# ChristophAl/tsne-flink

Hardware: AMD Instinct MI355X
Metric: t-SNE iterations/sec + end-to-end sec at N=1M×128 on 1/2/4/8 MI355X; kNN pts/s (higher is better)
Workload: dtype f64

## Files before the change

tsne-flink_amd/csrc/bhtree.hip:

```cpp
#include <hipcub/hipcub.hpp>

#include "bhtree_impl.hpp"

namespace tsne {
namespace {

constexpr int STACK = 320;
constexpr int QREC_V4 = sizeof(QRec) / 16;
constexpr int MOM_TASKS = 128;
__host__ __device__ constexpr double fact(int k) { return k <= 1 ? 1.0 : k * fact(k - 1); }
__host__ __device__ constexpr double binom(int k, int i) { return fact(k) / (fact(i) * fact(k - i)); }

__device__ __forceinline__ double recip_bh(double x) {
    const double r = __builtin_amdgcn_rcp(x);
    return __fma_rn(r, __fma_rn(-x, r, 1.0), r);
}

__device__ __forceinline__ void leaf_force(double qx, double qy, double px, double py, double &fx,
                                           double &fy, double &zs) {
    if (px == qx && py == qy) return;
    const double dx = qx - px, dy = qy - py;
    const double D = __fma_rn(dx, dx, dy * dy);
    const double r = recip_bh(1.0 + D);
    const double sc = r * r;
// ... 854 lines not shown
    }
    if (k == 0 && c == 0 && valid) {
        F[s] = make_double2(fx, fy);
        Z[s] = zs;
    }
    if (k == 0 && c == 0) nv.mtask_n[h * 64 + part * NQ + q] = valid ? ntask : 0;
    const int wwant = wave_sum(nwant);
    if (lane == 0) {
        nv.ncost[h * NPARTS + part] = npops + (ntilepts >> 6);
        if (wwant && __hip_atomic_load(&mom_flag[1], __ATOMIC_RELAXED, __HIP_MEMORY_SCOPE_AGENT) < mom_flag[2])
            atomicAdd(&mom_flag[1], wwant);
    }
    if (COST && bcost && __ballot(valid)) {
        const unsigned long long cc = ((unsigned long long)(clock64() - t_start) >> 6) + 1;
        if (cost_lab) {
            if (valid && k == 0 && c == 0) atomicAdd(&bcost[cost_lab[s] >> 8], (cc + NQ - 1) / NQ);
        } else {
            const int64_t sf = wave_min(valid ? s : ((int64_t)1 << 62));
            if (lane == 0) atomicAdd(&bcost[sf >> 8], cc);
        }
    }
    if (STATS && visits) {
        const unsigned long long tv = wave_sum(nvis);
        if (lane == 0) {
            atomicAdd(visits, tv);
            atomicAdd(visits + 3, (unsigned long long)npops);
            atomicAdd(visits + 4, (unsigned long long)ntilepts);
            atomicMax(visits + 8, (unsigned long long)npops);
            atomicAdd(visits + 30, 1ull);
            const unsigned long long w_end = wall_clock64();
            atomicMax(visits + 15, w_end - w_start);
            atomicMax(visits + 16, ~0ull - w_start);
            atomicMax(visits + 17, w_end);
            atomicAdd(visits + 18, w_end - w_start);
            atomicAdd(visits + 37, (unsigned long long)(clock64() - t_start));
            atomicMax(visits + 31, w_end - w_start);
            wave_log_put(nv.wlog, w_start, w_end, 1);
        }
    }
}

template <int MODE>
#ifdef NARROW_WPE
#define NARROW_ATTR __attribute__((amdgpu_waves_per_eu(NARROW_WPE)))
#else
#define NARROW_ATTR
#endif
__global__ __launch_bounds__(256) NARROW_ATTR void bh_traverse_narrow(
    const double2 *__restrict__ pos, const int32_t *__restrict__ dupc, const BHNode *__restrict__ nodes,
    const QRec *__restrict__ qrec, int32_t *__restrict__ ttask_n, const int32_t *__restrict__ meta,
    int32_t *__restrict__ mom_flag, double mom_tol, double theta, int64_t g0, int64_t g1,
    const int32_t *__restrict__ qlist, int32_t virt, double2 *__restrict__ F, double *__restrict__ Z,
// ... 1395 lines not shown
    val[b] = (int32_t)b;
}

int64_t narrow_fill(const tsne_ctx *ctx, int64_t waves) {
    const int64_t cap = 32 * (int64_t)ctx->cu_count;
    if (waves >= cap) return 0;
    return waves < cap / 2 ? waves : (cap - waves) / (NPARTS - 1);
}

}

static void block_order(tsne_ctx *ctx, BHTree &t, const int32_t *cost, int64_t nwaves, int64_t nblocks,
                        int32_t *order) {
    hipStream_t st = ctx->stream;
    hipLaunchKernelGGL(block_cost_keys, dim3(ceil_div(nblocks, 256)), dim3(256), 0, st, cost, nwaves, nblocks, t.okey,
                       t.oval);
    size_t tb = t.osort_tmp_bytes;
    TSNE_HIP(hipcub::DeviceRadixSort::SortPairsDescending(t.osort_tmp, tb, t.okey, t.okey2, t.oval, order,
                                                          (int)nblocks, 0, 32, st));
}

void bh_alloc(tsne_ctx *ctx, BHTree &t, int64_t n, const std::string &pre) {
    Workspace &ws = ctx->ws;
    bh_alloc_tree(ctx, t, n, pre);
    const int64_t qwaves = ceil_div(n, 64) + 4;
    t.tile_waves = qwaves + qwaves / 2 + 64;
    t.mtask = ws.get<int32_t>(pre + "mtask", (size_t)std::max<int64_t>(n, t.tile_waves * 64) * MOM_TASKS);
    t.mtask_n = ws.get<int32_t>(pre + "mtask_n", std::max<int64_t>(n, t.tile_waves * 64));
    t.ttask = ws.get<TileTask>(pre + "ttask", (size_t)t.tile_waves * TILE_CAP);
    t.ttask_n = ws.get<int32_t>(pre + "ttask_n", t.tile_waves);
    bh_alloc_build_tmp(ctx, t, n, pre);
    const int64_t nb = ceil_div(t.tile_waves, 4);
    t.wcost = ws.get<int32_t>(pre + "wcost", t.tile_waves);
    t.tcost = ws.get<int32_t>(pre + "tcost", t.tile_waves);
    t.okey = ws.get<int32_t>(pre + "okey", nb);
    t.okey2 = ws.get<int32_t>(pre + "okey2", nb);
    t.oval = ws.get<int32_t>(pre + "oval", nb);
    t.border = ws.get<int32_t>(pre + "border", nb);
    t.torder = ws.get<int32_t>(pre + "torder", nb);
    size_t ob = 0;
    TSNE_HIP(hipcub::DeviceRadixSort::SortPairsDescending(nullptr, ob, t.okey, t.okey2, t.oval, t.border, (int)nb, 0,
                                                          32, ctx->stream));
    t.osort_tmp_bytes = ob;
    t.osort_tmp = ws.get<uint8_t>(pre + "osort_tmp", ob);
    t.sel_waves = 0;
    t.ran_narrow = false;
// ... 86 lines not shown
    if (!t.sp_ctl) return 0;
    int32_t c[SP_NCTL];
    TSNE_HIP(hipMemcpyAsync(c, t.sp_ctl, sizeof(c), hipMemcpyDeviceToHost, ctx->stream));
    TSNE_HIP(hipStreamSynchronize(ctx->stream));
    return flags ? (int64_t)c[SP_OVF] : (int64_t)c[SP_TASKS];
}

int64_t bh_narrow_groups(tsne_ctx *ctx, BHTree &t) {
    if (!t.ran_narrow || !t.hran) return 0;
    int32_t h = 0;
    TSNE_HIP(hipMemcpyAsync(&h, t.hran, sizeof(int32_t), hipMemcpyDeviceToHost, ctx->stream));
    TSNE_HIP(hipStreamSynchronize(ctx->stream));
    return h;
}

BHTree &bh_single_tree(tsne_ctx *ctx, int64_t n) {
    if (!ctx->single_tree) ctx->single_tree = new BHTree();
    BHTree &t = *ctx->single_tree;
    if (t.n != n) bh_alloc(ctx, t, n, "bh1.");
    if (!ctx->opts.reuse_costs) { t.sel_waves = 0; t.sp_waves = 0; t.front_waves = 0; }
    return t;
}

void bh_repulsion(tsne_ctx *ctx, BHTree &t, double theta, int64_t s0, int64_t s1,
                  double2 *dF, double *dz, unsigned long long *visits, const int32_t *qlist,
                  unsigned long long *bcost, bool cost_by_label, int32_t *plim) {
    if (s1 <= s0) return;
    hipStream_t st = ctx->stream;
    const double mom_tol = ctx->opts.mom_tol;
    if (t.root_tile) {
        if (visits)
            hipLaunchKernelGGL(root_tile_eval<true>, dim3(ceil_div(s1 - s0, 256)), dim3(256), 0, st, t.root_pos,
                               t.nodes, t.rcoef, t.meta, s0, s1, qlist, dF, dz, visits, mom_tol);
        else
            hipLaunchKernelGGL(root_tile_eval<false>, dim3(ceil_div(s1 - s0, 256)), dim3(256), 0, st, t.root_pos,
                               t.nodes, t.rcoef, t.meta, s0, s1, qlist, dF, dz, visits, mom_tol);
        TSNE_LAUNCH_CHECK();
        return;
    }
    const int mode = visits ? 2 : (bcost ? 1 : 0);
    const bool burst = ctx->opts.trav_burst != 0;
    auto kern = plim ? (mode == 2 ? bh_traverse<2, true, false> : mode == 1 ? bh_traverse<1, true, false>
                                                                         : bh_traverse<0, true, false>)
                : burst ? (mode == 2 ? bh_traverse<2, false, false, true> : mode == 1 ? bh_traverse<1, false, false, true>
                                                                                   : bh_traverse<0, false, false, true>)
                        : (mode == 2 ? bh_traverse<2, false, false> : mode == 1 ? bh_traverse<1, false, false>
// ... 35 lines not shown
    const int cblocks = std::max(1, ctx->cu_count * o.tile_stream);
    if (stream) {
        bh_stream_alloc(ctx, t);
        stv.ctl = t.st_ctl;
        stv.gen = ++t.st_gen;
        if (t.st_gen >= (1 << 29)) t.st_gen = 1;
        stv.gen = t.st_gen;
        stv.maxcost = o.tile_stream_max;
        stv.wait = o.tile_stream_wait;
        stv.total = (int32_t)(nblocks * TRAV_WPB);
        stv.cap = (int32_t)t.tile_waves;
        if (!o.tile_stream_gate) {
            TSNE_HIP(hipEventRecord(ctx->st_ev[0], st));
            TSNE_HIP(hipStreamWaitEvent(ctx->st_stream, ctx->st_ev[0], 0));
        }
    }
    t.ran_stream = stream;
    bool mom_late = false;
    if (t.mom_deferred) {
        t.mom_deferred = false;
        if (stream) bh_moments(t, st);
        else mom_late = true;
    }
    if (mom_late && !narrow) {
        TSNE_HIP(hipEventRecord(ctx->aux_ev[0], st));
        TSNE_HIP(hipStreamWaitEvent(ctx->aux_stream, ctx->aux_ev[0], 0));
    }
    stv.prio = o.trav_prio;
    if (o.trav_front > 0.0 && narrow && t.front_waves == waves) stv.border = t.trav_order;
    if (t.order_ready && narrow && !plim && !qlist && s0 == 0 && waves == ceil_div(t.n, 64)) {
        TSNE_HIP(hipStreamWaitEvent(st, t.ord_ev, 0));
        stv.border = t.trav_order;
    }
    stv.wlog = wlog;
    const int32_t *clab = cost_by_label ? t.idx_sorted : nullptr;
    if (narrow) {
        TSNE_HIP(hipEventRecord(ctx->aux_ev[0], st));
        TSNE_HIP(hipStreamWaitEvent(ctx->aux_stream, ctx->aux_ev[0], 0));
        auto nk = mode == 2 ? bh_traverse_narrow<2> : mode == 1 ? bh_traverse_narrow<1> : bh_traverse_narrow<0>;
        hipLaunchKernelGGL(nk, dim3(nv.nbn), dim3(256), 0, ctx->aux_stream, t.pos, t.dupc, t.nodes, t.qrec, t.ttask_n,
                           t.meta, t.mom_flag, mom_tol, theta, s0, s1, qlist, (int32_t)t.n, dF, dz, visits, bcost,
                           t.tcost, clab, nv);
        TSNE_HIP(hipEventRecord(ctx->aux_ev[1], ctx->aux_stream));
    }
    hipLaunchKernelGGL(kern, dim3(nblocks), dim3(64 * TRAV_WPB), 0, st, t.pos, t.dupc, t.nodes, t.qrec, t.ttask, t.ttask_n,
                       t.meta, t.mom_flag, mom_tol, theta, s0, s1, qlist, (int32_t)t.n, dF, dz, visits, bcost, t.wcost,
                       t.tcost, clab, nv, plim, sv, stv);
    if (mom_late) {
        bh_moments(t, ctx->aux_stream);
        if (!t.mom_ev) TSNE_HIP(hipEventCreateWithFlags(&t.mom_ev, hipEventDisableTiming));
        TSNE_HIP(hipEventRecord(t.mom_ev, ctx->aux_stream));
    }
    if (stream) {
        if (o.tile_stream_gate)
            TSNE_HIP(hipStreamWaitValue32(ctx->st_stream, t.st_ctl + ST_STARTED, (uint32_t)nblocks,
                                          hipStreamWaitValueGte, 0xffffffffu));
        ChunkView scv;
        scv.Fp = t.st_Dp;
        scv.Zp = t.st_Dz;
        tile_apply_launch<2>(o.tile_pass, false, visits != nullptr, dim3(cblocks), ctx->st_stream, t.pos, t.nodes, t.ttask,
                             t.ttask_n, s0, s1, qlist, t.mom_flag, mom_tol, t.st_mtask, t.st_mtask_n, dF, dz, visits,
                             (const int32_t *)nullptr, scv, t.mom, SpillView(), stv, t.tcost);
        TSNE_HIP(hipEventRecord(ctx->st_ev[2], st));
        TSNE_HIP(hipStreamWaitEvent(ctx->st_stream, ctx->st_ev[2], 0));
        hipLaunchKernelGGL(stream_finish, dim3(ceil_div((int64_t)stv.total * 64, 256)), dim3(256), 0, ctx->st_stream,
                           t.pos, t.nodes, t.mom, t.st_ctl, t.st_mtask, t.st_mtask_n, t.st_Dp, t.st_Dz, s0, s1,
                           dF, dz, stv.cap, stv.gen);
        TSNE_HIP(hipMemsetAsync(t.st_ctl, 0, sizeof(int32_t) * ST_RESET, ctx->st_stream));
        TSNE_HIP(hipEventRecord(ctx->st_ev[1], ctx->st_stream));
    }
    const int levels = std::min(o.spill_drains, SP_LMAX);
    for (int d = 1; spill && d <= levels; ++d) {
        SpillView dv = sv;
        dv.lin = d;
        dv.lout = d < levels ? d + 1 : 0;
// ... 30 lines not shown
                         t.ttask_n, s0, s1, qlist, t.mom_flag, mom_tol, t.mtask, t.mtask_n, dF, dz, visits, torder, cv,
                         t.mom, SpillView(), stv, t.tcost);
    hipLaunchKernelGGL(moment_apply, dim3(ceil_div(tslots * 64, 256)), dim3(256), 0, st, t.pos, t.nodes, t.mom,
                       t.mtask, t.mtask_n, s0, s1, qlist, dF, dz, cv);
    const bool keep_pcost = o.trav_front_cur > 0.0 && !plim && !qlist && s0 == 0 && s1 == t.n;
    if (keep_pcost) {
        t.pcost = ctx->ws.get<int32_t>(t.pre + "pcost", (size_t)t.n);
        t.pred = ctx->ws.get<int32_t>(t.pre + "pred", (size_t)ceil_div(t.n, 64) + 1);
        t.trav_order = ctx->ws.get<int32_t>(t.pre + "trav_order", ceil_div(t.tile_waves, TRAV_WPB) + 1);
    }
    hipLaunchKernelGGL(chunk_combine, dim3(ceil_div(s1 - s0, 256)), dim3(256), 0, st, t.ch_Fp, t.ch_Zp, t.ch_C,
                       t.ch_slot0, s0, s1, qlist, dF, dz, keep_pcost ? t.pcost : nullptr, t.idx_sorted, t.wcost,
                       narrow ? t.nflag : nullptr);
    t.pcost_valid = keep_pcost;
    if (spill) {
        tile_apply_launch<1>(o.tile_pass, false, visits != nullptr, dim3(std::max(1, ctx->cu_count * 4)), st, t.pos, t.nodes,
                             t.ttask, t.ttask_n, s0, s1, qlist, t.mom_flag, mom_tol, t.mtask, t.mtask_n, dF, dz, visits,
                             (const int32_t *)nullptr, ChunkView(), t.mom, sv, StreamView(), t.tcost);
        hipLaunchKernelGGL(spill_combine, dim3(ceil_div(s1 - s0, 256)), dim3(256), 0, st, t.sp_gflag, t.sp_gen,
                           t.sp_acc, s0, s1, qlist, dF, dz, t.sp_ctl);
    }
    if (narrow) {
        TSNE_HIP(hipStreamWaitEvent(st, ctx->aux_ev[1], 0));
        hipLaunchKernelGGL(narrow_moment_apply, dim3(ceil_div(t.nar_hmax * 64, 256)), dim3(256), 0, st, t.pos,
                           t.nodes, t.mom, t.hlist, t.hcount, t.nmtask, t.nmtask_n, s0, s1, qlist, dF, dz);
        TSNE_HIP(hipMemcpyAsync(t.hran, t.hcount, sizeof(int32_t), hipMemcpyDeviceToDevice, st));
    }
    if (nfac > 0.0 && !plim) {
        if (!narrow) TSNE_HIP(hipMemsetAsync(t.nflag, 0, sizeof(int32_t) * waves, st));
        const bool front = o.trav_front > 0.0;
        if (front) t.trav_order = ctx->ws.get<int32_t>(t.pre + "trav_order", ceil_div(t.tile_waves, TRAV_WPB) + 1);
        hipLaunchKernelGGL(narrow_select, dim3(1), dim3(1024), 0, st, t.wcost, waves, t.nflag, t.ncost, t.hlist,
                           t.hcount, t.nar_hmax, nfac, std::min<int64_t>(t.nar_hmax, narrow_fill(ctx, waves)),
                           front ? t.trav_order : nullptr, o.trav_front);
        t.sel_waves = waves;
        t.front_waves = front ? waves : 0;
    } else {
        t.sel_waves = 0;
        t.front_waves = 0;
    }
    if (o.spill > 0.0 && o.spill_force == 0 && !plim) {
        bh_spill_alloc(ctx, t);
        hipLaunchKernelGGL(spill_budget, dim3(1), dim3(1024), 0, st, t.wcost, waves, o.spill, o.spill_task,
                           (int32_t)o.spill_min, t.sp_ctl);
        t.sp_waves = waves;
    } else {
        t.sp_waves = 0;
    }
    if (stream) TSNE_HIP(hipStreamWaitEvent(st, ctx->st_ev[1], 0));
    TSNE_LAUNCH_CHECK();
}

bool repulsion_stat(tsne_ctx *ctx, const std::string &name, int64_t *value_out) {
    const int at = name == "bh.pops" ? 3 : name == "bh.tile_points" ? 4 : name == "bh.child_slots" ? 6
                 : name == "bh.visits" ? 0 : name == "bh.wave_ticks_max" ? 15 : name == "bh.wave_ticks_sum" ? 18
                 : name == "bh.span_ticks" ? 17 : name == "bh.dense_pairs" ? 2 : name == "bh.moment_evals" ? 1
                 : name == "bh.tile_ticks_max" ? 19 : name == "bh.tile_ticks_sum" ? 22 : name == "bh.tile_span_ticks" ? 21
                 : name == "bh.slow_wave_ticks" ? 33 : name == "bh.slow_wave_pops" ? 33 : name == "bh.slow_wave_ties" ? 34
                 : name == "bh.slow_wave_tile_points" ? 35 : name == "bh.slow_wave_slots" ? 36
                 : name == "bh.wave_mhz" ? 37 : -1;
    int atk = at;
    if (at < 0 && name.size() == 14 && name.compare(0, 13, "bh.tile_steps") == 0) atk = 24 + 2 * (name[13] - '0');
    if (at < 0 && name.size() == 14 && name.compare(0, 13, "bh.tile_pairs") == 0) atk = 25 + 2 * (name[13] - '0');
    if (at < 0 && name.size() == 17 && name.compare(0, 14, "bh.tile_gsteps") == 0 && name[15] == '_' &&
        (name[14] == '0' || name[14] == '1') && (name[16] == '2' || name[16] == '4' || name[16] == '8'))
        atk = (name[14] == '1' ? 38 : 41) + (name[16] == '2' ? 0 : name[16] == '4' ? 1 : 2);
    if (name == "bh.tile_rounds_max") atk = 44;
    if (name == "bh.tile_chunked_waves") atk = 45;
    if (atk < 0 || atk >= VIS_N) return false;
    TSNE_REQUIRE(ctx->opts.rep_stats && ctx->ws.has("rep.visits"), "counter '" + name + "' needs option rep_stats");
    unsigned long long v[VIS_N];
    TSNE_HIP(hipMemcpyAsync(v, ctx->ws.get<unsigned long long>("rep.visits", VIS_N), sizeof(v), hipMemcpyDeviceToHost,
                            ctx->stream));
    TSNE_HIP(hipStreamSynchronize(ctx->stream));
    *value_out = atk == 17 ? (int64_t)(v[17] - (~0ull - v[16])) : atk == 21 ? (int64_t)(v[21] - (~0ull - v[20]))
                                                                              : (int64_t)v[atk];
    if (atk == 37) *value_out = v[18] ? (int64_t)(100.0 * (double)v[37] / (double)v[18]) : 0;
    if (atk >= 33 && atk <= 36)
        *value_out = name == "bh.slow_wave_ticks" ? (int64_t)(v[atk] >> 24) : (int64_t)(v[atk] & ((1ull << 24) - 1));
    return true;
}

}
```

tsne-flink_amd/csrc/bhtree.hpp:

```cpp
#pragma once
#include "common.hpp"
#include "csort.hpp"

namespace tsne {

constexpr int TILE_CAP = 8192;
struct TileTask {
    int32_t ref, first, last, pad;
    uint64_t mask;
};

struct __attribute__((aligned(16))) BHNode {
    double cx, cy;
    double h;
    double hmin;
    double bx0, bx1, by0, by1;
    int32_t cnt;
    int32_t left;
    int32_t right;
    int32_t delta;
    int32_t first, last;
    double rball;
};

// ... 100 lines not shown
    int4 *sp_task = nullptr;
    uint4 *sp_ent = nullptr;
    int32_t *sp_gflag = nullptr;
    unsigned long long *sp_acc = nullptr;
    TileTask *sp_pg_tiles = nullptr;
    int32_t *sp_pg_grp = nullptr, *sp_pg_n = nullptr;
    int32_t sp_cap = 0, sp_pg_cap = 0;
    int32_t sp_gen = 0;
    int64_t sp_waves = 0;
    bool ran_spill = false;
    int32_t *st_ctl = nullptr;
    double2 *st_Dp = nullptr;
    double *st_Dz = nullptr;
    int32_t *st_mtask = nullptr, *st_mtask_n = nullptr;
    int32_t st_gen = 0;
    size_t st_words = 0;
    int32_t *trav_order = nullptr;
    int64_t front_waves = 0;
    int32_t *pcost = nullptr, *pred = nullptr;
    bool pcost_valid = false, order_ready = false;
    hipEvent_t ord_ev = nullptr;
    bool mom_deferred = false;
    hipEvent_t mom_ev = nullptr;
    bool ran_stream = false;
    std::string pre;
};

void bh_alloc(tsne_ctx *ctx, BHTree &t, int64_t n, const std::string &pre = "bh.");
BHTree &bh_single_tree(tsne_ctx *ctx, int64_t n);
void bh_build(tsne_ctx *ctx, BHTree &t, const double *dY, double theta, const int32_t *rowmap = nullptr,
              bool root_tile_ok = false, double near_tol = -1.0);
double bh_near_tol(const tsne_ctx *ctx, bool late);
void bh_repulsion(tsne_ctx *ctx, BHTree &t, double theta, int64_t s0, int64_t s1,
                  double2 *dF, double *dz, unsigned long long *visits, const int32_t *qlist = nullptr,
                  unsigned long long *bcost = nullptr, bool cost_by_label = false, int32_t *plim = nullptr);
void part_align(tsne_ctx *ctx, BHTree &t, const int64_t *cuts, int world, int rank, int32_t *plim);
void part_recut(tsne_ctx *ctx, const unsigned long long *cost, int world, int64_t n, int64_t *cuts);
void part_cost(tsne_ctx *ctx, BHTree &t, int64_t waves, unsigned long long *out);
int64_t bh_spill_counter(tsne_ctx *ctx, BHTree &t, bool flags);
int64_t bh_stream_counter(tsne_ctx *ctx, BHTree &t);
int64_t bh_narrow_groups(tsne_ctx *ctx, BHTree &t);
void bh_balance(tsne_ctx *ctx, const unsigned long long *bcost, int64_t n, int world, int64_t *bounds);

}
```

tsne-flink_amd/csrc/bhtree_build.hip:

```cpp
#include <hipcub/hipcub.hpp>

#include "bhtree_impl.hpp"

namespace tsne {
namespace {

constexpr uint64_t OUT_KEY = MORTON2_OUT_KEY;
constexpr int MOM_CHUNK = 2048;

__global__ void bbox_partial(const double *__restrict__ Y, int64_t n, double *__restrict__ part) {
    __shared__ double sm[4][4];
    double mnx = __builtin_inf(), mxx = -__builtin_inf(), mny = __builtin_inf(), mxy = -__builtin_inf();
    for (int64_t i = (int64_t)blockIdx.x * blockDim.x + threadIdx.x; i < n;
         i += (int64_t)gridDim.x * blockDim.x) {
        double x = Y[2 * i], y = Y[2 * i + 1];
        mnx = fmin(mnx, x); mxx = fmax(mxx, x);
        mny = fmin(mny, y); mxy = fmax(mxy, y);
    }
    mnx = wave_min(mnx); mxx = wave_max(mxx); mny = wave_min(mny); mxy = wave_max(mxy);
    const int w = threadIdx.x >> 6;
    if (lane_id() == 0) { sm[w][0] = mnx; sm[w][1] = mxx; sm[w][2] = mny; sm[w][3] = mxy; }
    __syncthreads();
    if (threadIdx.x == 0) {
        for (int k = 1; k < 4; ++k) {
// ... 1019 lines not shown
    t.status_h = ctx->pinned;
    t.rcoef = ws.get<double>(pre + "rcoef", POLY_K);
    t.dup_mask = ((uint64_t)1 << (64 - __builtin_clzll((uint64_t)std::max<int64_t>(2, 4 * n) - 1))) - 1;
    t.dup_tab = ws.get<int32_t>(pre + "dup_tab", t.dup_mask + 1);
    t.dup_open = ws.get<uint8_t>(pre + "dup_open", n);
    size_t tb = 0;
    morton_sort(nullptr, tb, t.keys, t.keys_sorted, t.idx, t.idx_sorted, n, ctx->stream);
    t.sort_tmp_bytes = tb;
    t.sort_tmp = ws.get<uint8_t>(pre + "sort_tmp", tb);
    csort_alloc(ctx, t.cs, n, pre);
    t.cs_primed = false;
}

double bh_near_tol(const tsne_ctx *ctx, bool late) { return late ? ctx->opts.near_tol_late : ctx->opts.near_tol_early; }

double bh_near_dmax(double theta, double tol) {
    if (!(theta > 0.0)) return __builtin_inf();
    if (!(tol > 0.0)) return -1.0;
    double d = std::sqrt(tol / (48.0 * theta * theta));
    while (48.0 * theta * theta * d * d * (1.0 + 8.0 * d) > tol) d *= 0.99;
    return d;
}

void bh_moments(BHTree &t, hipStream_t ms) {
    const int64_t n = t.n;
    hipLaunchKernelGGL(moment_count, dim3(ceil_div(n + 1, 1024)), dim3(1024), 0, ms, t.nodes, n, t.meta, t.mom_flag,
                       t.mom_cnt, t.mom_list, t.meta, t.mom_off, t.mom_item);
    const int mgrid = (int)std::min<int64_t>(2048, std::max<int64_t>(1, ceil_div(n, 256)));
    hipLaunchKernelGGL(moment_items<true>, dim3(mgrid), dim3(256), 0, ms, t.pos, t.nodes, t.mom_off, n, t.mom_item,
                       t.mom_part, t.mom_cnt, t.mom);
    hipLaunchKernelGGL(moment_reduce, dim3(mgrid), dim3(256), 0, ms, t.meta, t.mom_list, t.mom_cnt, t.mom_off,
                       t.mom_part, t.mom);
}

void bh_build(tsne_ctx *ctx, BHTree &t, const double *dY, double theta, const int32_t *rowmap, bool root_tile_ok,
              double near_tol) {
    if (near_tol < 0.0) near_tol = bh_near_tol(ctx, false);
    t.near_dmax = bh_near_dmax(theta, near_tol);
    hipStream_t st = ctx->stream;
    const int64_t n = t.n;
    t.rowmap = rowmap;
    t.root_tile = false;
    t.mom_deferred = false;
    const bool fuse_opt = ctx->opts.build_fuse != 0;
    if (!fuse_opt) TSNE_HIP(hipMemsetAsync(t.dflag, 0, sizeof(int32_t), st));
    hipLaunchKernelGGL(bbox_partial, dim3(t.bbox_blocks), dim3(256), 0, st, dY, n, t.bbox_part);
    hipLaunchKernelGGL(bbox_final, dim3(1), dim3(256), 0, st, t.bbox_part, t.bbox_blocks, t.W, t.meta, t.bb,
                       t.mom_flag, t.mom_off + n, fuse_opt ? t.dflag : nullptr);
    if (root_tile_ok && t.rt_skip > 0) {
        --t.rt_skip;
        root_tile_ok = false;
    }
    if (root_tile_ok) {
        hipLaunchKernelGGL(root_tile_check, dim3(1), dim3(1), 0, st, t.dflag, t.bb, t.W, n, theta, t.near_dmax,
                           t.status);
        TSNE_HIP(hipMemcpyAsync(t.status_h, t.status, 2 * sizeof(int32_t), hipMemcpyDeviceToHost, st));
        TSNE_HIP(hipStreamSynchronize(st));
        if (!t.status_h[0]) {
            root_tile_ok = false;
            if (t.status_h[1] >= 3) t.rt_skip = std::min(64, 4 * (t.status_h[1] - 2));
        }
    }
    if (root_tile_ok) {
// ... 92 lines not shown
```

tsne-flink_amd/csrc/bhtree_impl.hpp:

```cpp
#pragma once

#include "bhtree.hpp"

namespace tsne {
namespace {

constexpr int MOM_ORDER = 4;
constexpr int MOM_DEG = 2 * MOM_ORDER + 1;
constexpr int MOM_K = (MOM_DEG + 1) * (MOM_DEG + 2) / 2;
constexpr int MOM_MIN_POINTS = 64;
__host__ __device__ constexpr int midx(int a, int b) { return a * (MOM_DEG + 1) - a * (a - 1) / 2 + b; }

__host__ __device__ constexpr int poly_len(int d) { return (d + 1) * (d + 2) / 2; }
__host__ __device__ constexpr int poly_off_z(int i) { return i == 0 ? 0 : poly_off_z(i - 1) + poly_len(2 * i - 2); }
constexpr int POLY_X = poly_off_z(MOM_ORDER + 1);
__host__ __device__ constexpr int poly_off_x(int i) { return i == 0 ? POLY_X : poly_off_x(i - 1) + poly_len(2 * i - 1); }
constexpr int POLY_Y = poly_off_x(MOM_ORDER + 1);
__host__ __device__ constexpr int poly_off_y(int i) { return POLY_Y + poly_off_x(i) - POLY_X; }
constexpr int POLY_K = POLY_Y + (POLY_Y - POLY_X);
static_assert(POLY_K == 345, "MOM_ORDER 4: 95 + 125 + 125 coefficients");

#ifndef TRAV_WPB
#define TRAV_WPB 4
#endif

constexpr int32_t REF_FORCED = 1 << 30;
constexpr int PART_LEVEL = 10;

__device__ __forceinline__ void box_centre(double bx0, double bx1, double by0, double by1, double &cx, double &cy,
                                           double &R) {
    cx = 0.5 * (bx0 + bx1);
    cy = 0.5 * (by0 + by1);
    const double ex = 0.5 * (bx1 - bx0), ey = 0.5 * (by1 - by0);
    R = sqrt(ex * ex + ey * ey) * (1.0 + 1e-12);
}
__device__ __forceinline__ void box_centre(const BHNode &nd, double &cx, double &cy, double &R) {
    box_centre(nd.bx0, nd.bx1, nd.by0, nd.by1, cx, cy, R);
}

}

void bh_moments(BHTree &t, hipStream_t ms);

void bh_alloc_tree(tsne_ctx *ctx, BHTree &t, int64_t n, const std::string &pre);
void bh_alloc_build_tmp(tsne_ctx *ctx, BHTree &t, int64_t n, const std::string &pre);

}
```

tsne-flink_amd/csrc/capi.cpp:

```cpp
#include <cmath>
#include <cstdio>
#include <cstring>
#include <exception>
#include <new>
#include <algorithm>
#include <thread>

#include "bhtree.hpp"
#include "common.hpp"
#include "pca.hpp"
#include "ranks.hpp"
#include "transform.hpp"

namespace tsne {

static thread_local std::string g_last_error;

[[noreturn]] void fail(int status, const std::string &msg) { throw Error(status, msg); }

template <class Fn> static int guard(Fn &&fn) {
    try {
        fn();
        return TSNE_OK;
    } catch (const Error &e) {
// ... 100 lines not shown
    {"spill", &Options::spill, nullptr, 0.0, 1e6},
    {"spill_task", &Options::spill_task, nullptr, 0.0, 1e6},
    {"spill_min", nullptr, &Options::spill_min, 1, 1 << 30},
    {"spill_force", nullptr, &Options::spill_force, 0, 1 << 30},
    {"spill_drains", nullptr, &Options::spill_drains, 1, 8},
    {"tile_stream", nullptr, &Options::tile_stream, 0, 8},
    {"tile_stream_max", nullptr, &Options::tile_stream_max, -1, 1 << 30},
    {"tile_stream_frac", &Options::tile_stream_frac, nullptr, 0.0, 64.0},
    {"tile_stream_gate", nullptr, &Options::tile_stream_gate, 0, 1},
    {"trav_prio", nullptr, &Options::trav_prio, 0, 3},
    {"trav_burst", nullptr, &Options::trav_burst, 0, 1},
    {"trav_front", &Options::trav_front, nullptr, 0.0, 1e6},
    {"trav_front_cur", &Options::trav_front_cur, nullptr, 0.0, 1e6},
    {"wave_log", nullptr, &Options::wave_log, 0, 1},
    {"attract_serial_t0", nullptr, &Options::attract_serial_t0, 0, 1 << 30},
    {"attract_serial_t1", nullptr, &Options::attract_serial_t1, -1, 1 << 30},
    {"tile_stream_wait", nullptr, &Options::tile_stream_wait, 1, 1 << 20},
    {"comm_world1", nullptr, &Options::comm_world1, 0, 1},
    {"rep_stats", nullptr, &Options::rep_stats, 0, 1},
    {"loop_serial", nullptr, &Options::loop_serial, 0, 1},
    {"bu_acqrel", nullptr, &Options::bu_acqrel, 0, 1},
    {"bh_split", nullptr, &Options::bh_split, 0, 1},
    {"build_fuse", nullptr, &Options::build_fuse, 0, 1},
    {"tile_pass", nullptr, &Options::tile_pass, 0, 8},
    {"tile_prefetch", nullptr, &Options::tile_prefetch, 0, 1},
    {"transform_resort", nullptr, &Options::transform_resort, 0, 1 << 30},
    {"transform_split", nullptr, &Options::transform_split, 0, 1},
    {"transform_stats", nullptr, &Options::transform_stats, 0, 1},
};
static const OptionField &option_field(const char *key) {
    for (const OptionField &f : k_options)
        if (std::strcmp(f.key, key) == 0) return f;
    fail(TSNE_ERR_ARG, std::string("unknown option '") + key + "'");
}
static void set_option(Options &o, const char *key, double v) {
    const OptionField &f = option_field(key);
    TSNE_REQUIRE(v >= f.lo && v <= f.hi, std::string("option '") + key + "' out of range");
    if (f.d) o.*f.d = v;
    else {
        TSNE_REQUIRE(v == std::floor(v), std::string("option '") + key + "' takes an integer");
        TSNE_REQUIRE(f.i != &Options::tile_pass || v <= 2 || v == 4 || v == 8, "option 'tile_pass' takes 0, 1, 2, 4 or 8");
        o.*f.i = (int)v;
    }
}
static double get_option(const Options &o, const char *key) {
    const OptionField &f = option_field(key);
// ... 109 lines not shown
        TSNE_REQUIRE(d_bcost != nullptr && d_bounds != nullptr && n >= 0 && world >= 1, "bad balance arguments");
        bh_balance(ctx, reinterpret_cast<const unsigned long long *>(d_bcost), n, world, d_bounds);
    });
}

int tsne_ctx_create(int32_t device, tsne_ctx **out) {
    return guard([&] {
        TSNE_REQUIRE(out != nullptr, "out is NULL");
        *out = nullptr;
        int count = 0;
        if (hipGetDeviceCount(&count) != hipSuccess || count <= 0)
            fail(TSNE_ERR_NO_DEVICE, "no HIP device visible");
        TSNE_REQUIRE(device >= 0 && device < count, "device index out of range");
        TSNE_HIP(hipSetDevice(device));
        hipDeviceProp_t prop;
        TSNE_HIP(hipGetDeviceProperties(&prop, device));
        std::unique_ptr<tsne_ctx> c(new tsne_ctx());
        c->device = device;
        c->cu_count = prop.multiProcessorCount;
        TSNE_HIP(hipStreamCreateWithFlags(&c->stream, hipStreamNonBlocking));
        c->own_stream = true;
        TSNE_HIP(hipStreamCreateWithFlags(&c->aux_stream, hipStreamNonBlocking));
        for (auto &e : c->aux_ev) TSNE_HIP(hipEventCreateWithFlags(&e, hipEventDisableTiming));
        TSNE_HIP(hipHostMalloc(reinterpret_cast<void **>(&c->pinned), 64 * sizeof(int32_t)));
        *out = c.release();
    });
}

int tsne_ctx_create_multi(const int32_t *devices, int32_t ndev, tsne_ctx **out) {
    return guard([&] {
        TSNE_REQUIRE(out != nullptr, "out is NULL");
        *out = nullptr;
        TSNE_REQUIRE(devices != nullptr && ndev >= 1 && ndev <= 64, "bad device list");
        bool same = true, distinct = true;
        for (int a = 0; a < ndev; ++a)
            for (int b = a + 1; b < ndev; ++b) {
                if (devices[a] == devices[b]) distinct = false;
                else same = false;
            }
        TSNE_REQUIRE(same || distinct, "devices must be all distinct (RCCL) or all the same (loopback ranks)");
        std::unique_ptr<tsne_ctx> g(new tsne_ctx());
        struct Undo {
            tsne_ctx *g;
            ~Undo() { if (g) for (tsne_ctx *c : g->group) tsne_ctx_destroy(c); }
        } undo{g.get()};
        for (int r = 0; r < ndev; ++r) {
// ... 5 lines not shown
        g->device = devices[0];
        g->cu_count = g->group[0]->cu_count;
        comm_init_group(g->group, same && ndev > 1);
        g->world = ndev;
        undo.g = nullptr;
        *out = g.release();
    });
}

int tsne_ctx_destroy(tsne_ctx *ctx) {
    if (!ctx) return TSNE_OK;
    if (!ctx->group.empty()) {
        int rc = TSNE_OK;
        for (tsne_ctx *c : ctx->group) {
            const int r = tsne_ctx_destroy(c);
            if (rc == TSNE_OK) rc = r;
        }
        delete ctx;
        return rc;
    }
    int rc = guard([&] {
        DeviceGuard g(ctx->device);
        (void)hipStreamSynchronize(ctx->stream);
        opt_destroy(ctx);
        transform_destroy(ctx);
        delete ctx->single_tree;
        ctx->single_tree = nullptr;
        comm_destroy(ctx);
        ctx->timers.clear();
        ctx->ws.clear();
        if (ctx->pinned) (void)hipHostFree(ctx->pinned);
        ctx->pinned = nullptr;
        if (ctx->own_stream && ctx->stream) (void)hipStreamDestroy(ctx->stream);
        if (ctx->aux_stream) (void)hipStreamSynchronize(ctx->aux_stream);
        if (ctx->aux_stream) (void)hipStreamDestroy(ctx->aux_stream);
        for (auto &e : ctx->aux_ev)
            if (e) (void)hipEventDestroy(e);
        if (ctx->st_stream) (void)hipStreamSynchronize(ctx->st_stream);
        if (ctx->st_stream) (void)hipStreamDestroy(ctx->st_stream);
        for (auto &e : ctx->st_ev)
            if (e) (void)hipEventDestroy(e);
    });
    delete ctx;
    return rc;
}

int tsne_ctx_set_stream(tsne_ctx *ctx, void *hip_stream) {
    return guard([&] {
        check_ctx(ctx);
        ctx = primary(ctx);
        DeviceGuard g(ctx->device);
        if (ctx->own_stream && ctx->stream) {
            TSNE_HIP(hipStreamSynchronize(ctx->stream));
            TSNE_HIP(hipStreamDestroy(ctx->stream));
        }
        if (hip_stream) {
            ctx->stream = static_cast<hipStream_t>(hip_stream);
            ctx->own_stream = false;
// ... 1007 lines not shown
```

tsne-flink_amd/csrc/common.hpp:

```cpp
#pragma once

#include <hip/hip_runtime.h>

#include <cstdint>
#include <cstring>
#include <deque>
#include <map>
#include <memory>
#include <stdexcept>
#include <string>
#include <vector>

#include "../../include/tsne_hip.h"

namespace tsne {

struct Error : std::runtime_error {
    int status;
    Error(int s, const std::string &m) : std::runtime_error(m), status(s) {}
};

[[noreturn]] void fail(int status, const std::string &msg);

#define TSNE_HIP(expr)                                                                     \
// ... 143 lines not shown
    int attract_stream = 1;
    int graph_order = 1;
    int relabel = -1;
    int recut = 0;
    int knn_bf16 = 1;
    double narrow = 3.0;
    int bh_split = 0;
    int bu_acqrel = 1;
    int loop_serial = 0;
    int rep_stats = 0;
    int comm_world1 = 0;
    int reuse_costs = 0;
    double spill = 0.0, spill_task = 0.25;
    int spill_min = 256, spill_force = 0, spill_drains = 2;
    int tile_stream = 0, tile_stream_max = 0;
    double tile_stream_frac = 1.0;
    int tile_stream_wait = 48;
    int attract_serial_t0 = 0, attract_serial_t1 = -1;
    int wave_log = 0;
    double trav_front = 0.0;
    double trav_front_cur = 0.0;
    int trav_prio = 0;
    int trav_burst = 1;
    int tile_stream_gate = 1;
    int transform_resort = 10;
    int transform_split = 0;
    int transform_stats = 0;
};

}

struct tsne_ctx {
    int device = 0;
    hipStream_t stream = nullptr;
    bool own_stream = false;
    hipStream_t aux_stream = nullptr;
    hipEvent_t aux_ev[2] = {nullptr, nullptr};
    hipStream_t st_stream = nullptr;
    hipEvent_t st_ev[3] = {nullptr, nullptr, nullptr};
    int rank = 0, world = 1;
    tsne::Comm *comm = nullptr;
    tsne::Workspace ws;
    tsne::OptState *opt = nullptr;
    tsne::Options opts;
    tsne::BHTree *single_tree = nullptr;
    tsne::BHTree *query_tree = nullptr;
    tsne::OctTree *query_tree3 = nullptr;
    tsne::TransformState *xform = nullptr;
    std::string loop_profile_pending;
    tsne::StageTimers timers;
    int32_t *pinned = nullptr;
    int cu_count = 256;
    int64_t knn_fallback_queries = 0;
    int64_t quality_fallbacks[2] = {0, 0};
    std::vector<tsne_ctx *> group;
};

namespace tsne {

struct DeviceGuard {
// ... 139 lines not shown
```

tsne-flink_amd/csrc/optimize.hip:

```cpp
#include <hipcub/hipcub.hpp>

#include "attract.hpp"
#include "bhtree.hpp"
#include "octree.hpp"

namespace tsne {

struct OptState {
    tsne_params p{};
    int C = 2;
    int64_t n = 0, nnz = 0;
    double *Yu = nullptr, *updu = nullptr, *gainsu = nullptr;
    int64_t *rp0 = nullptr;
    int32_t *col0 = nullptr;
    double *val0 = nullptr;
    int64_t *rpw = nullptr;
    int32_t *colw = nullptr;
    double *valw = nullptr;
    double *Y[2] = {nullptr, nullptr}, *upd[2] = {nullptr, nullptr}, *gains[2] = {nullptr, nullptr};
    int32_t *orig[2] = {nullptr, nullptr};
    int32_t *lab = nullptr;
    int cur = 0;
    std::vector<int64_t> own;
    int64_t L0 = 0, L1 = 0;
// ... 579 lines not shown
    if (want_loss) {
        hipLaunchKernelGGL(reduce_partial, dim3(NPART), dim3(256), 0, st, lpart, blocks, 1, 0, part);
        hipLaunchKernelGGL(reduce_final, dim3(1), dim3(256), 0, st, part, NPART, scal + 1, 0.0);
    }
    double hs[2] = {0, 0};
    TSNE_HIP(hipMemcpyAsync(hs, scal, 2 * sizeof(double), hipMemcpyDeviceToHost, st));
    TSNE_HIP(hipStreamSynchronize(st));
    if (h_sumq) *h_sumq = hs[0];
    if (h_loss) *h_loss = hs[1];
}


void opt_destroy(tsne_ctx *ctx) {
    if (!ctx->opt) return;
    OptState *s = ctx->opt;
    for (auto &e : s->ev)
        if (e) (void)hipEventDestroy(e);
    for (hipEvent_t e : {s->ev_y, s->ev_attr})
        if (e) (void)hipEventDestroy(e);
    if (s->side) {
        (void)hipStreamSynchronize(s->side);
        (void)hipStreamDestroy(s->side);
    }
    delete ctx->opt;
    ctx->opt = nullptr;
}

static std::vector<int64_t> equal_cuts(int64_t n, int world) {
    std::vector<int64_t> c(world + 1);
    const int64_t chunk = ceil_div(n, world);
    for (int r = 0; r <= world; ++r) c[r] = std::min<int64_t>(n, chunk * r);
    return c;
}

static void gather_working_set(tsne_ctx *ctx, OptState *s) {
    if (!sharded(ctx)) return;
    const int c = s->cur;
    std::vector<int64_t> off(ctx->world + 1);
    for (int r = 0; r <= ctx->world; ++r) off[r] = s->own[r] * s->C * (int64_t)sizeof(double);
    comm_allgatherv(ctx, s->upd[c], off.data());
    comm_allgatherv(ctx, s->gains[c], off.data());
}

static void build_own_rows(tsne_ctx *ctx, OptState *s) {
    hipStream_t st = ctx->stream;
    const int64_t m = s->L1 - s->L0;
// ... 603 lines not shown
```

Baseline: 218.7.

## Chain narrow moment apply and selection onto aux stream, moments on own stream

Adds a bh_chain option, on by default, that reschedules BH repulsion work across streams. Deferred moment computation gets its own stream with a smaller moment_count block size. narrow_moment_apply now runs on the aux stream right after moments instead of on the main stream. The narrow_select pass is offloaded to the aux stream and joined lazily at the next build or alloc. The intent is to overlap these small serial kernels with the main traversal and cut main-stream idle gaps, at the cost of extra events, stream synchronization and more complex ordering. It also adds a narrow-moment-task stats counter and BHTree event cleanup.

```diff
diff --git a/tsne-flink_amd/csrc/bhtree.hip b/tsne-flink_amd/csrc/bhtree.hip
--- a/tsne-flink_amd/csrc/bhtree.hip
+++ b/tsne-flink_amd/csrc/bhtree.hip
@@ -900,12 +900,14 @@
     }
     if (STATS && visits) {
         const unsigned long long tv = wave_sum(nvis);
+        const unsigned long long tn = wave_sum((unsigned long long)(k == 0 && c == 0 && valid ? ntask : 0));
         if (lane == 0) {
             atomicAdd(visits, tv);
             atomicAdd(visits + 3, (unsigned long long)npops);
             atomicAdd(visits + 4, (unsigned long long)ntilepts);
             atomicMax(visits + 8, (unsigned long long)npops);
             atomicAdd(visits + 30, 1ull);
+            atomicAdd(visits + 46, tn);
             const unsigned long long w_end = wall_clock64();
             atomicMax(visits + 15, w_end - w_start);
             atomicMax(visits + 16, ~0ull - w_start);
@@ -2347,6 +2349,7 @@
 
 void bh_alloc(tsne_ctx *ctx, BHTree &t, int64_t n, const std::string &pre) {
     Workspace &ws = ctx->ws;
+    bh_select_join(ctx, t);
     bh_alloc_tree(ctx, t, n, pre);
     const int64_t qwaves = ceil_div(n, 64) + 4;
     t.tile_waves = qwaves + qwaves / 2 + 64;
@@ -2479,6 +2482,16 @@
     return t;
 }
 
+void bh_select_join(tsne_ctx *ctx, BHTree &t) {
+    if (!t.sel_pending) return;
+    t.sel_pending = false;
+    TSNE_HIP(hipStreamWaitEvent(ctx->stream, t.sel_ev, 0));
+}
+
+#ifndef MOM_COUNT_CHAIN
+#define MOM_COUNT_CHAIN 256
+#endif
+
 void bh_repulsion(tsne_ctx *ctx, BHTree &t, double theta, int64_t s0, int64_t s1,
                   double2 *dF, double *dz, unsigned long long *visits, const int32_t *qlist,
                   unsigned long long *bcost, bool cost_by_label, int32_t *plim) {
@@ -2560,9 +2573,13 @@
         if (stream) bh_moments(t, st);
         else mom_late = true;
     }
+    const bool chain = o.bh_chain != 0 && o.tile_stream == 0 && o.spill <= 0.0 && o.spill_force == 0 &&
+                       !(o.trav_front_cur > 0.0);
+    const bool mom_own = mom_late && chain && ctx->mom_stream;
+    const hipStream_t mst = mom_own ? ctx->mom_stream : ctx->aux_stream;
     if (mom_late && !narrow) {
         TSNE_HIP(hipEventRecord(ctx->aux_ev[0], st));
-        TSNE_HIP(hipStreamWaitEvent(ctx->aux_stream, ctx->aux_ev[0], 0));
+        if (!mom_own) TSNE_HIP(hipStreamWaitEvent(ctx->aux_stream, ctx->aux_ev[0], 0));
     }
     stv.prio = o.trav_prio;
     if (o.trav_front > 0.0 && narrow && t.front_waves == waves) stv.border = t.trav_order;
@@ -2579,16 +2596,26 @@
         hipLaunchKernelGGL(nk, dim3(nv.nbn), dim3(256), 0, ctx->aux_stream, t.pos, t.dupc, t.nodes, t.qrec, t.ttask_n,
                            t.meta, t.mom_flag, mom_tol, theta, s0, s1, qlist, (int32_t)t.n, dF, dz, visits, bcost,
                            t.tcost, clab, nv);
-        TSNE_HIP(hipEventRecord(ctx->aux_ev[1], ctx->aux_stream));
+        if (!chain) TSNE_HIP(hipEventRecord(ctx->aux_ev[1], ctx->aux_stream));
     }
     hipLaunchKernelGGL(kern, dim3(nblocks), dim3(64 * TRAV_WPB), 0, st, t.pos, t.dupc, t.nodes, t.qrec, t.ttask, t.ttask_n,
                        t.meta, t.mom_flag, mom_tol, theta, s0, s1, qlist, (int32_t)t.n, dF, dz, visits, bcost, t.wcost,
                        t.tcost, clab, nv, plim, sv, stv);
     if (mom_late) {
-        bh_moments(t, ctx->aux_stream);
+        if (mom_own) TSNE_HIP(hipStreamWaitEvent(mst, ctx->aux_ev[0], 0));
+        bh_moments(t, mst, mom_own ? MOM_COUNT_CHAIN : 1024);
         if (!t.mom_ev) TSNE_HIP(hipEventCreateWithFlags(&t.mom_ev, hipEventDisableTiming));
-        TSNE_HIP(hipEventRecord(t.mom_ev, ctx->aux_stream));
-    }
+        TSNE_HIP(hipEventRecord(t.mom_ev, mst));
+    }
+    if (chain && narrow) {
+        if (mom_late) TSNE_HIP(hipStreamWaitEvent(ctx->aux_stream, t.mom_ev, 0));
+        hipLaunchKernelGGL(narrow_moment_apply, dim3(ceil_div(t.nar_hmax * 64, 256)), dim3(256), 0, ctx->aux_stream, t.pos,
+                           t.nodes, t.mom, t.hlist, t.hcount, t.nmtask, t.nmtask_n, s0, s1, qlist, dF, dz);
+        TSNE_HIP(hipMemcpyAsync(t.hran, t.hcount, sizeof(int32_t), hipMemcpyDeviceToDevice, ctx->aux_stream));
+        TSNE_HIP(hipEventRecord(ctx->aux_ev[1], ctx->aux_stream));
+    }
+    const bool sel_off = chain && nfac > 0.0 && !plim;
+    if (sel_off) TSNE_HIP(hipEventRecord(ctx->aux_ev[2], st));
     if (stream) {
         if (o.tile_stream_gate)
             TSNE_HIP(hipStreamWaitValue32(ctx->st_stream, t.st_ctl + ST_STARTED, (uint32_t)nblocks,
@@ -2665,17 +2692,26 @@
     }
     if (narrow) {
         TSNE_HIP(hipStreamWaitEvent(st, ctx->aux_ev[1], 0));
-        hipLaunchKernelGGL(narrow_moment_apply, dim3(ceil_div(t.nar_hmax * 64, 256)), dim3(256), 0, st, t.pos,
-                           t.nodes, t.mom, t.hlist, t.hcount, t.nmtask, t.nmtask_n, s0, s1, qlist, dF, dz);
-        TSNE_HIP(hipMemcpyAsync(t.hran, t.hcount, sizeof(int32_t), hipMemcpyDeviceToDevice, st));
+        if (!chain) {
+            hipLaunchKernelGGL(narrow_moment_apply, dim3(ceil_div(t.nar_hmax * 64, 256)), dim3(256), 0, st, t.pos,
+                               t.nodes, t.mom, t.hlist, t.hcount, t.nmtask, t.nmtask_n, s0, s1, qlist, dF, dz);
+            TSNE_HIP(hipMemcpyAsync(t.hran, t.hcount, sizeof(int32_t), hipMemcpyDeviceToDevice, st));
+        }
     }
     if (nfac > 0.0 && !plim) {
-        if (!narrow) TSNE_HIP(hipMemsetAsync(t.nflag, 0, sizeof(int32_t) * waves, st));
+        const hipStream_t ss = sel_off ? ctx->aux_stream : st;
+        if (sel_off) TSNE_HIP(hipStreamWaitEvent(ss, ctx->aux_ev[2], 0));
+        if (!narrow) TSNE_HIP(hipMemsetAsync(t.nflag, 0, sizeof(int32_t) * waves, ss));
         const bool front = o.trav_front > 0.0;
         if (front) t.trav_order = ctx->ws.get<int32_t>(t.pre + "trav_order", ceil_div(t.tile_waves, TRAV_WPB) + 1);
-        hipLaunchKernelGGL(narrow_select, dim3(1), dim3(1024), 0, st, t.wcost, waves, t.nflag, t.ncost, t.hlist,
+        hipLaunchKernelGGL(narrow_select, dim3(1), dim3(1024), 0, ss, t.wcost, waves, t.nflag, t.ncost, t.hlist,
                            t.hcount, t.nar_hmax, nfac, std::min<int64_t>(t.nar_hmax, narrow_fill(ctx, waves)),
                            front ? t.trav_order : nullptr, o.trav_front);
+        if (sel_off) {
+            if (!t.sel_ev) TSNE_HIP(hipEventCreateWithFlags(&t.sel_ev, hipEventDisableTiming));
+            TSNE_HIP(hipEventRecord(t.sel_ev, ss));
+            t.sel_pending = true;
+        }
         t.sel_waves = waves;
         t.front_waves = front ? waves : 0;
     } else {
@@ -2710,6 +2746,7 @@
         atk = (name[14] == '1' ? 38 : 41) + (name[16] == '2' ? 0 : name[16] == '4' ? 1 : 2);
     if (name == "bh.tile_rounds_max") atk = 44;
     if (name == "bh.tile_chunked_waves") atk = 45;
+    if (name == "bh.narrow_moment_tasks") atk = 46;
     if (atk < 0 || atk >= VIS_N) return false;
     TSNE_REQUIRE(ctx->opts.rep_stats && ctx->ws.has("rep.visits"), "counter '" + name + "' needs option rep_stats");
     unsigned long long v[VIS_N];
diff --git a/tsne-flink_amd/csrc/bhtree.hpp b/tsne-flink_amd/csrc/bhtree.hpp
--- a/tsne-flink_amd/csrc/bhtree.hpp
+++ b/tsne-flink_amd/csrc/bhtree.hpp
@@ -146,6 +146,15 @@
     hipEvent_t ord_ev = nullptr;
     bool mom_deferred = false;
     hipEvent_t mom_ev = nullptr;
+    hipEvent_t sel_ev = nullptr;
+    bool sel_pending = false;
+    BHTree() = default;
+    BHTree(const BHTree &) = delete;
+    BHTree &operator=(const BHTree &) = delete;
+    ~BHTree() {
+        for (hipEvent_t e : {ord_ev, mom_ev, sel_ev})
+            if (e) (void)hipEventDestroy(e);
+    }
     bool ran_stream = false;
     std::string pre;
 };
@@ -155,6 +164,7 @@
 void bh_build(tsne_ctx *ctx, BHTree &t, const double *dY, double theta, const int32_t *rowmap = nullptr,
               bool root_tile_ok = false, double near_tol = -1.0);
 double bh_near_tol(const tsne_ctx *ctx, bool late);
+void bh_select_join(tsne_ctx *ctx, BHTree &t);
 void bh_repulsion(tsne_ctx *ctx, BHTree &t, double theta, int64_t s0, int64_t s1,
                   double2 *dF, double *dz, unsigned long long *visits, const int32_t *qlist = nullptr,
                   unsigned long long *bcost = nullptr, bool cost_by_label = false, int32_t *plim = nullptr);
diff --git a/tsne-flink_amd/csrc/bhtree_build.hip b/tsne-flink_amd/csrc/bhtree_build.hip
--- a/tsne-flink_amd/csrc/bhtree_build.hip
+++ b/tsne-flink_amd/csrc/bhtree_build.hip
@@ -1065,10 +1065,10 @@
     return d;
 }
 
-void bh_moments(BHTree &t, hipStream_t ms) {
+void bh_moments(BHTree &t, hipStream_t ms, int count_threads) {
     const int64_t n = t.n;
-    hipLaunchKernelGGL(moment_count, dim3(ceil_div(n + 1, 1024)), dim3(1024), 0, ms, t.nodes, n, t.meta, t.mom_flag,
-                       t.mom_cnt, t.mom_list, t.meta, t.mom_off, t.mom_item);
+    hipLaunchKernelGGL(moment_count, dim3(ceil_div(n + 1, count_threads)), dim3(count_threads), 0, ms, t.nodes, n, t.meta,
+                       t.mom_flag, t.mom_cnt, t.mom_list, t.meta, t.mom_off, t.mom_item);
     const int mgrid = (int)std::min<int64_t>(2048, std::max<int64_t>(1, ceil_div(n, 256)));
     hipLaunchKernelGGL(moment_items<true>, dim3(mgrid), dim3(256), 0, ms, t.pos, t.nodes, t.mom_off, n, t.mom_item,
                        t.mom_part, t.mom_cnt, t.mom);
@@ -1082,6 +1082,7 @@
     t.near_dmax = bh_near_dmax(theta, near_tol);
     hipStream_t st = ctx->stream;
     const int64_t n = t.n;
+    bh_select_join(ctx, t);
     t.rowmap = rowmap;
     t.root_tile = false;
     t.mom_deferred = false;
diff --git a/tsne-flink_amd/csrc/bhtree_impl.hpp b/tsne-flink_amd/csrc/bhtree_impl.hpp
--- a/tsne-flink_amd/csrc/bhtree_impl.hpp
+++ b/tsne-flink_amd/csrc/bhtree_impl.hpp
@@ -40,7 +40,7 @@
 
 }
 
-void bh_moments(BHTree &t, hipStream_t ms);
+void bh_moments(BHTree &t, hipStream_t ms, int count_threads = 1024);
 
 void bh_alloc_tree(tsne_ctx *ctx, BHTree &t, int64_t n, const std::string &pre);
 void bh_alloc_build_tmp(tsne_ctx *ctx, BHTree &t, int64_t n, const std::string &pre);
diff --git a/tsne-flink_amd/csrc/capi.cpp b/tsne-flink_amd/csrc/capi.cpp
--- a/tsne-flink_amd/csrc/capi.cpp
+++ b/tsne-flink_amd/csrc/capi.cpp
@@ -146,6 +146,7 @@
     {"bu_acqrel", nullptr, &Options::bu_acqrel, 0, 1},
     {"bh_split", nullptr, &Options::bh_split, 0, 1},
     {"build_fuse", nullptr, &Options::build_fuse, 0, 1},
+    {"bh_chain", nullptr, &Options::bh_chain, 0, 1},
     {"tile_pass", nullptr, &Options::tile_pass, 0, 8},
     {"tile_prefetch", nullptr, &Options::tile_prefetch, 0, 1},
     {"transform_resort", nullptr, &Options::transform_resort, 0, 1 << 30},
@@ -301,6 +302,7 @@
         c->own_stream = true;
         TSNE_HIP(hipStreamCreateWithFlags(&c->aux_stream, hipStreamNonBlocking));
         for (auto &e : c->aux_ev) TSNE_HIP(hipEventCreateWithFlags(&e, hipEventDisableTiming));
+        TSNE_HIP(hipStreamCreateWithFlags(&c->mom_stream, hipStreamNonBlocking));
         TSNE_HIP(hipHostMalloc(reinterpret_cast<void **>(&c->pinned), 64 * sizeof(int32_t)));
         *out = c.release();
     });
@@ -352,6 +354,8 @@
     int rc = guard([&] {
         DeviceGuard g(ctx->device);
         (void)hipStreamSynchronize(ctx->stream);
+        if (ctx->aux_stream) (void)hipStreamSynchronize(ctx->aux_stream);
+        if (ctx->mom_stream) (void)hipStreamSynchronize(ctx->mom_stream);
         opt_destroy(ctx);
         transform_destroy(ctx);
         delete ctx->single_tree;
@@ -364,6 +368,8 @@
         if (ctx->own_stream && ctx->stream) (void)hipStreamDestroy(ctx->stream);
         if (ctx->aux_stream) (void)hipStreamSynchronize(ctx->aux_stream);
         if (ctx->aux_stream) (void)hipStreamDestroy(ctx->aux_stream);
+        if (ctx->mom_stream) (void)hipStreamSynchronize(ctx->mom_stream);
+        if (ctx->mom_stream) (void)hipStreamDestroy(ctx->mom_stream);
         for (auto &e : ctx->aux_ev)
             if (e) (void)hipEventDestroy(e);
         if (ctx->st_stream) (void)hipStreamSynchronize(ctx->st_stream);
diff --git a/tsne-flink_amd/csrc/common.hpp b/tsne-flink_amd/csrc/common.hpp
--- a/tsne-flink_amd/csrc/common.hpp
+++ b/tsne-flink_amd/csrc/common.hpp
@@ -189,6 +189,7 @@
     double trav_front_cur = 0.0;
     int trav_prio = 0;
     int trav_burst = 1;
+    int bh_chain = 1;
     int tile_stream_gate = 1;
     int transform_resort = 10;
     int transform_split = 0;
@@ -202,7 +203,8 @@
     hipStream_t stream = nullptr;
     bool own_stream = false;
     hipStream_t aux_stream = nullptr;
-    hipEvent_t aux_ev[2] = {nullptr, nullptr};
+    hipEvent_t aux_ev[3] = {nullptr, nullptr, nullptr};
+    hipStream_t mom_stream = nullptr;
     hipStream_t st_stream = nullptr;
     hipEvent_t st_ev[3] = {nullptr, nullptr, nullptr};
     int rank = 0, world = 1;
diff --git a/tsne-flink_amd/csrc/optimize.hip b/tsne-flink_amd/csrc/optimize.hip
--- a/tsne-flink_amd/csrc/optimize.hip
+++ b/tsne-flink_amd/csrc/optimize.hip
@@ -625,6 +625,7 @@
         (void)hipStreamSynchronize(s->side);
         (void)hipStreamDestroy(s->side);
     }
+    if (ctx->aux_stream) (void)hipStreamSynchronize(ctx->aux_stream);
     delete ctx->opt;
     ctx->opt = nullptr;
 }
```

Result: faster. 221.6, median of 6 (+1.3%).
